# franioli/icepy4d

Measured on AMD Instinct MI355X. Metric: matched stereo image-pairs/sec (4096 kpts, 1080p), higher is better.
Workload: dtype f32

## Files before the change

icepy4d_amd/csrc/attention_bx.hip:

```cpp
#include "bf16x3.h"
#include "common.h"
#include "kernels.h"

namespace im {

static constexpr int BKT = 32;
static constexpr int BKS = 144;
static constexpr int BVS = 192;
static constexpr int BK_PLANE = BKT * BKS, BV_PLANE = BKT * BVS;
static constexpr int B_STAGE = 3 * BK_PLANE + 3 * BV_PLANE;
static constexpr int B_LDS = 2 * B_STAGE;
static constexpr int DPL = BKT * 128;
static constexpr int D_LDS = 3 * 3 * (DPL + DPL);

__device__ __forceinline__ f32x16 mfma_attn(u32x4 a, u32x4 b, f32x16 c) {
#ifdef BX_ABL_NO_MFMA
    c[0] += __uint_as_float(a.x ^ b.x);
    return c;
#else
    return mfma_bf(a, b, c);
#endif
}

typedef __attribute__((address_space(3))) bf16x4 lds_bf16x4;
// ... 449 lines not shown
        sc = sn;
        { const int rr = r0; r0 = r1; r1 = r2; r2 = RD == 3 ? rr : r0; }
        __syncthreads();
    }
    if (a.clock && nt > 8) {
        const unsigned long long ck1 = __builtin_amdgcn_s_memtime(), cr1 = __builtin_amdgcn_s_memrealtime();
        if (threadIdx.x == 0) {
            unsigned long long* cp = a.clock + 2 * (blockIdx.x % CLOCK_PROBE_SLOTS);
            cp[0] = ck1 - ck0; cp[1] = cr1 - cr0;
        }
    }
    {
        const int t = nt - 1;
        m_use = softmax_ref<true>(sc, t * BKT, nk, hh, m_run, l_run, o0, o1);
        softmax_exp(sc, m_use, l_run);
        pv_mul(r0, sc);
    }

    if (n_split > 1) {
        const long prow = (((long)z * a.heads + head) * a.n_max + min(qrow, a.n_max - 1)) * 66;
        const long pstride = (long)a.batch * a.heads * a.n_max * 66;
        float* pp = a.part + (long)split * pstride + prow;
        if (qrow < nq) {
#pragma unroll
            for (int g = 0; g < 4; ++g) {
                *reinterpret_cast<float2*>(pp + 8 * g + 4 * hh) = make_float2(o0[4 * g], o0[4 * g + 1]);
                *reinterpret_cast<float2*>(pp + 8 * g + 4 * hh + 2) = make_float2(o0[4 * g + 2], o0[4 * g + 3]);
                *reinterpret_cast<float2*>(pp + 32 + 8 * g + 4 * hh) = make_float2(o1[4 * g], o1[4 * g + 1]);
                *reinterpret_cast<float2*>(pp + 32 + 8 * g + 4 * hh + 2) = make_float2(o1[4 * g + 2], o1[4 * g + 3]);
            }
            if (hh == 0) { pp[64] = m_run; pp[65] = l_run; }
        }
        __threadfence();
        __syncthreads();
        int* flag = reinterpret_cast<int*>(bsm);
        if (tid == 0) {
            int* cnt = a.counters + ((long)z * a.heads + head) * nqb + qblk;
            const int old = atomicAdd(cnt, 1);
            *flag = (old == n_split - 1);
            if (old == n_split - 1) *cnt = 0;
        }
        __syncthreads();
        if (!*flag) return;
        __threadfence();
        float m = -INFINITY;
        for (int sidx = 0; sidx < n_split; ++sidx) m = fmaxf(m, a.part[(long)sidx * pstride + prow + 64]);
        l_run = 0.f;
#pragma unroll
        for (int r = 0; r < 16; ++r) { o0[r] = 0.f; o1[r] = 0.f; }
        for (int sidx = 0; sidx < n_split; ++sidx) {
            const float* ps = a.part + (long)sidx * pstride + prow;
            const float w = __builtin_amdgcn_exp2f(ps[64] - m);
            l_run += w * ps[65];
#pragma unroll
            for (int g = 0; g < 4; ++g)
#pragma unroll
                for (int q = 0; q < 4; ++q) {
                    o0[4 * g + q] += w * ps[8 * g + 4 * hh + q];
                    o1[4 * g + q] += w * ps[32 + 8 * g + 4 * hh + q];
                }
        }
    }

    if (qrow < nq) {
        const float inv = 1.f / l_run;
        float* op = a.out + (long)z * a.out_bstride + (long)qrow * a.ldo + head * 64;
#pragma unroll
        for (int g = 0; g < 4; ++g) {
            const float4 w0 = make_float4(o0[4 * g] * inv, o0[4 * g + 1] * inv, o0[4 * g + 2] * inv, o0[4 * g + 3] * inv);
            const float4 w1 = make_float4(o1[4 * g] * inv, o1[4 * g + 1] * inv, o1[4 * g + 2] * inv, o1[4 * g + 3] * inv);
            *reinterpret_cast<float4*>(op + 8 * g + 4 * hh) = w0;
            *reinterpret_cast<float4*>(op + 32 + 8 * g + 4 * hh) = w1;
        }
    }
}

hipError_t launch_attn_planes(const AttnArgs& a, hipStream_t s) {
    if (!a.planes || a.n_max <= 0 || attn_f32_form(a)) return hipSuccess;
    const long rows = (long)a.batch * a.heads * a.n_max;
    hipLaunchKernelGGL(kv_planes_kernel, dim3((unsigned)((rows + 31) / 32), 2), dim3(256), 0, s, a);
    return hipGetLastError();
}

hipError_t launch_flash_attn_bx(const AttnArgs& a, hipStream_t s) {
    const dim3 grid(((a.n_max + 127) / 128) * a.heads * a.batch * (a.part ? ATTN_MAX_SPLIT : 1)), block(256);
    static const bool reg_staging = env_int("IM_ATTN_REG_STAGING") != 0;
    if (a.planes && !reg_staging) return launch_dyn_lds<flash_attn_bx_kernel<true, true>>(grid, block, D_LDS, s, a);
    if (a.planes) return launch_dyn_lds<flash_attn_bx_kernel<true, false>>(grid, block, B_LDS, s, a);
    return launch_dyn_lds<flash_attn_bx_kernel<false, false>>(grid, block, B_LDS, s, a);
}

}
```

icepy4d_amd/csrc/block.h:

```cpp
#pragma once
#include "ctx.h"

namespace im {

struct BlockFfn {
    int act = 0;
    const float* w0 = nullptr; const float* w0p = nullptr;
    const float* b0 = nullptr;
    const float* ln_g = nullptr; const float* ln_b = nullptr;
    const float* w3 = nullptr; const float* w3p = nullptr;
    const float* b3 = nullptr;
    const char* name_fused = nullptr; const char* name_ffn0 = nullptr; const char* name_ffn3 = nullptr;
};

int launch_block_proj(im_ctx* ctx, hipStream_t s, const char* name, const GemmArgs& g, const float* wp_layers, int layer);

int launch_block_tail(im_ctx* ctx, hipStream_t s, const AttnArgs& at, const BlockFfn& f, const GemmArgs& base, float* x);

}
```

icepy4d_amd/csrc/block.hip:

```cpp
#include "block.h"

#include "lg_misc.h"
#include "workspace.h"

namespace im {

int launch_block_proj(im_ctx* ctx, hipStream_t s, const char* name, const GemmArgs& g, const float* wp_layers, int layer) {
    if (env_is_1("IM_PROJ_TILED")) {
        IM_LAUNCH(ctx, name, s, launch_gemm(g, s));
        return 0;
    }
    GemmArgs r = g;
    r.wp = reinterpret_cast<const unsigned char*>(wp_layers) + (size_t)layer * g.N * 256 * 6;
    IM_LAUNCH(ctx, name, s, launch_proj_rows(r, s));
    return 0;
}

int launch_block_tail(im_ctx* ctx, hipStream_t s, const AttnArgs& at, const BlockFfn& f, const GemmArgs& base, float* x) {
    Workspace* ws = ctx->ws;
    const long xb = (long)base.m_max * 256, hb = (long)base.m_max * 512;
    IM_LAUNCH(ctx, "attn_kv_planes", s, launch_attn_planes(at, s));
    IM_LAUNCH(ctx, at.cross ? "flash_attn_cross" : "flash_attn_self", s, launch_flash_attn(at, s));
    static const bool unfused = env_is_1("IM_FFN_UNFUSED");
    if (!unfused) {
        FfnArgs a;
        a.act = f.act; a.x = x; a.x_bstride = xb; a.att = at.out; a.att_bstride = xb;
        a.w0p = f.w0p; a.b0 = f.b0; a.ln_g = f.ln_g; a.ln_b = f.ln_b; a.w3p = f.w3p; a.b3 = f.b3;
        a.m_max = base.m_max; a.batch = base.batch; a.m_ptr = base.m_ptr; a.active = base.active; a.pstride = base.pstride;
        IM_LAUNCH(ctx, f.name_fused, s, launch_ffn_fused(a, s));
        return 0;
    }
    {
        GemmArgs g = base;
        g.A = x; g.a_bstride = xb; g.lda = 256; g.A1 = at.out; g.a1_bstride = xb; g.lda1 = 256; g.ksplit = 256;
        g.W = f.w0; g.ldw = 512; g.bias = f.b0; g.N = 512; g.K = 512;
        g.C = ws->h; g.c_bstride = hb; g.ldc = 512; g.epi = f.act == 1 ? EPI_BIAS_RELU : EPI_BIAS;
        IM_LAUNCH(ctx, f.name_ffn0, s, launch_gemm(g, s));
    }
    if (f.act == 0)
        IM_LAUNCH(ctx, "lg_layernorm_gelu", s, launch_layernorm_gelu(ws->h, hb, ws->st, base.batch, base.m_max, f.ln_g, f.ln_b, s));
    {
        GemmArgs g = base;
        g.A = ws->h; g.a_bstride = hb; g.lda = 512; g.W = f.w3; g.ldw = 512; g.bias = f.b3; g.N = 256; g.K = 512;
        g.C = x; g.c_bstride = xb; g.ldc = 256; g.R = x; g.r_bstride = xb; g.ldr = 256; g.epi = EPI_BIAS_RESID;
        IM_LAUNCH(ctx, f.name_ffn3, s, launch_gemm(g, s));
    }
    return 0;
}

}
```

icepy4d_amd/csrc/capi.hip:

```cpp
#include "ctx.h"
#include "lg_misc.h"
#include "sp_post.h"
#include "workspace.h"

#include <algorithm>
#include <cstdio>
#include <cstdlib>
#include <cstring>

using namespace im;

template <int N, typename F>
static hipError_t with_uploads(const float* const (&src)[N], const size_t (&sizes)[N], hipStream_t st, F&& launch) {
    float* d[N] = {};
    hipError_t e = hipSuccess;
    for (int i = 0; i < N && e == hipSuccess; ++i) {
        e = hipMalloc(&d[i], sizes[i] * sizeof(float));
        if (e == hipSuccess) e = hipMemcpy(d[i], src[i], sizes[i] * sizeof(float), hipMemcpyHostToDevice);
    }
    if (e == hipSuccess) e = launch(d);
    const hipError_t e2 = hipStreamSynchronize(st);
    for (int i = 0; i < N; ++i) hipFree(d[i]);
    return e != hipSuccess ? e : e2;
}
// ... 83 lines not shown
    ws->sim_ps = (((size_t)K * K + (size_t)K + 4) + 3) & ~(size_t)3;
    ws->vec_ps = ((size_t)K + 4 + 3) & ~(size_t)3;
    ws->part_ps = (size_t)((K + 15) / 16 + 1) * (K + 4);
    A(ws->sim, NP * ws->sim_ps + (size_t)K + 8);
    A(ws->sim2, (size_t)1);
    A(ws->rmax, NP * ws->vec_ps); A(ws->rlog, NP * ws->vec_ps); A(ws->cmax, NP * ws->vec_ps); A(ws->clog, NP * ws->vec_ps);
    A(ws->part, NP * ws->part_ps);
    A(ws->ridx, NP * ws->vec_ps); A(ws->rval, NP * ws->vec_ps); A(ws->cbest, NP * ws->vec_ps);
    A(ws->st, NP); A(ws->sel, NP + 3);
    A(ws->uv, (size_t)4 * (K + 8));
#undef A
    ws->n_pairs = (int)NP;
    if (!ok) {
        for (void* p : ws->allocs) ctx->gfree(p);
        delete ws;
        ctx->max_h = ctx->max_w = ctx->max_images = ctx->max_kpts = 0;
        return ctx->fail(-31, "im_ctx_reserve: out of device memory (%d x %d, %d images, %d keypoints)", max_h, max_w, max_images, max_kpts);
    }
    ctx->ws = ws;
    ctx->max_h = max_h; ctx->max_w = max_w; ctx->max_images = max_images; ctx->max_kpts = max_kpts;
    IM_HIP(ctx, hipMemset(ws->st, 0, sizeof(LGState) * NP));
    IM_HIP(ctx, hipMemset(ws->sel, 0, (NP + 3) * sizeof(int)));
    IM_HIP(ctx, hipMemset(ws->attn_cnt, 0, attn_counter_ints((int)K, (int)NI, 4) * sizeof(int)));
    IM_HIP(ctx, hipDeviceSynchronize());
    return 0;
}

int im_profile_begin(im_ctx* ctx) {
    IM_CHECK_CTX(ctx);
    IM_HIP(ctx, hipDeviceSynchronize());
    for (auto& e : ctx->prof) { ctx->prof_pool.push_back(e.e0); ctx->prof_pool.push_back(e.e1); }
    ctx->prof.clear();
    ctx->prof_on = true;
    return 0;
}

int im_profile_end(im_ctx* ctx, char* buf, size_t cap) {
    IM_CHECK_CTX(ctx);
    ctx->prof_on = false;
    constexpr int NCAL = 32;
    hipEvent_t cal[2 * NCAL];
    for (int i = 0; i < NCAL; ++i) {
        cal[2 * i] = ctx->prof_event(); cal[2 * i + 1] = ctx->prof_event();
        hipEventRecord(cal[2 * i], ctx->prof_stream);
        hipEventRecord(cal[2 * i + 1], ctx->prof_stream);
    }
    IM_HIP(ctx, hipDeviceSynchronize());
    std::map<std::string, std::pair<int, double>> agg;
    for (int i = 0; i < NCAL; ++i) {
        float ms = 0.f;
        if (hipEventElapsedTime(&ms, cal[2 * i], cal[2 * i + 1]) == hipSuccess) { agg["_empty_event_pair"].first += 1; agg["_empty_event_pair"].second += ms; }
        ctx->prof_pool.push_back(cal[2 * i]); ctx->prof_pool.push_back(cal[2 * i + 1]);
    }
    for (auto& e : ctx->prof) {
        float ms = 0.f;
        IM_HIP(ctx, hipEventElapsedTime(&ms, e.e0, e.e1));
        auto& a = agg[e.name];
        a.first += 1;
        a.second += ms;
    }
    std::string out = "{";
    bool first = true;
    for (auto& kv : agg) {
        char line[256];
        snprintf(line, sizeof(line), "%s\"%s\": {\"count\": %d, \"total_ms\": %.6f}", first ? "" : ", ", kv.first.c_str(),
                 kv.second.first, kv.second.second);
        out += line;
        first = false;
    }
    out += "}";
    if (!buf || out.size() + 1 > cap) return ctx->fail(-60, "im_profile_end: buffer too small (%zu needed)", out.size() + 1);
    memcpy(buf, out.c_str(), out.size() + 1);
    return 0;
}

int im_debug_read(im_ctx* ctx, const char* name, float* d_dst, size_t nfloats, void* stream) {
    IM_CHECK_CTX(ctx);
    Workspace* ws = ctx->ws;
    if (!ws || !name) return ctx->fail(-51, "im_debug_read: no workspace");
    const size_t K = (size_t)ctx->max_kpts;
    const std::string nm = name;
    const float* src = nullptr;
    size_t avail = 0;
    if (nm == "lg_x") { src = ws->x[ctx->dbg_cur]; avail = 2 * K * 256; }
    else if (nm == "lg_cos") { src = ws->cs[ctx->dbg_cur]; avail = 2 * K * 32; }
    else if (nm == "lg_sin") { src = ws->sn[ctx->dbg_cur]; avail = 2 * K * 32; }
    else if (nm == "sim") { src = ws->sim; avail = K * K; }
    else if (nm == "md") { src = ws->md; avail = 2 * K * 256; }
    else if (nm == "sp_smap") { src = ws->smap; avail = ws->smap_floats; }
    else if (nm == "sp_nms") { src = ws->nms; avail = ws->smap_floats; }
    else return ctx->fail(-61, "im_debug_read: unknown buffer '%s'", name);
    if (nfloats > avail) return ctx->fail(-62, "im_debug_read: %zu floats requested, %zu available", nfloats, avail);
    IM_HIP(ctx, hipMemcpyAsync(d_dst, src, nfloats * sizeof(float), hipMemcpyDeviceToDevice, (hipStream_t)stream));
    IM_HIP(ctx, hipStreamSynchronize((hipStream_t)stream));
    return 0;
}

int im_debug_clock_probe(im_ctx* ctx, int arm, double* h_out, void* stream) {
    IM_CHECK_CTX(ctx);
    hipStream_t s = (hipStream_t)stream;
    const size_t bytes = (size_t)CLOCK_PROBE_SLOTS * 2 * sizeof(unsigned long long);
    if (arm == 1) {
        IM_GROW(ctx, ctx->grow(ctx->scratch.clock[0], bytes, "clock_probe_attention"), -22, "im_debug_clock_probe: allocation failed");
        IM_GROW(ctx, ctx->grow(ctx->scratch.clock[1], bytes, "clock_probe_convolution"), -22, "im_debug_clock_probe: allocation failed");
        IM_HIP(ctx, hipMemsetAsync(ctx->scratch.clock[0].p, 0, bytes, s));
        IM_HIP(ctx, hipMemsetAsync(ctx->scratch.clock[1].p, 0, bytes, s));
        IM_HIP(ctx, hipStreamSynchronize(s));
        ctx->clock_armed = true;
        return 0;
    }
    if (!ctx->scratch.clock[0].p || !h_out) return ctx->fail(-51, "im_debug_clock_probe: not armed");
    std::vector<unsigned long long> h((size_t)CLOCK_PROBE_SLOTS * 2);
    const void* src[2] = {ctx->scratch.clock[0].p, ctx->scratch.clock[1].p};
    for (int c = 0; c < 2; ++c) {
        IM_HIP(ctx, hipMemcpyAsync(h.data(), src[c], bytes, hipMemcpyDeviceToHost, s));
        IM_HIP(ctx, hipStreamSynchronize(s));
        std::vector<double> mhz;
        for (int i = 0; i < CLOCK_PROBE_SLOTS; ++i)
            if (h[2 * i + 1] > 0) mhz.push_back(100.0 * (double)h[2 * i] / (double)h[2 * i + 1]);
        std::sort(mhz.begin(), mhz.end());
        h_out[2 * c] = mhz.empty() ? 0.0 : mhz[mhz.size() / 2];
        h_out[2 * c + 1] = (double)mhz.size();
    }
    if (arm == 0) ctx->clock_armed = false;
    return 0;
}

int im_gemm_nt(im_ctx* ctx, const float* d_a, const float* d_w, const float* d_bias, float* d_c, int m, int n, int k,
               float alpha, int big_tile, void* stream) {
    IM_CHECK_CTX(ctx);
    GemmArgs g;
    g.A = d_a; g.lda = k; g.W = d_w; g.ldw = k; g.bias = d_bias; g.N = n; g.K = k; g.m_max = m;
    g.C = d_c; g.ldc = n; g.alpha = alpha; g.epi = EPI_BIAS; g.big_tile = big_tile & 1; g.bx = (big_tile >> 1) & 1;
    IM_HIP(ctx, launch_gemm(g, (hipStream_t)stream));
    return 0;
}

int im_ffn_fused(im_ctx* ctx, int act, float* d_x, const float* d_att, const float* h_w0, const float* h_b0, const float* h_ln_g,
                   const float* h_ln_b, const float* h_w3, const float* h_b3, int n_images, int n_rows, const int32_t* d_n, void* stream) {
    IM_CHECK_CTX(ctx);
    if (n_images < 1 || n_rows < 1 || act < 0 || act > 1 || (act == 0 && (!h_ln_g || !h_ln_b))) return ctx->fail(-12, "im_ffn_fused: bad arguments");
    if (act == 1) h_ln_g = h_ln_b = h_b0;
    const std::vector<float> p0 = pack_frag_weights(h_w0, 512, 512), p3 = pack_frag_weights(h_w3, 256, 512);
    const size_t sizes[6] = {p0.size(), 512, 512, 512, p3.size(), 256};
    const float* src[6] = {p0.data(), h_b0, h_ln_g, h_ln_b, p3.data(), h_b3};
    hipStream_t st = (hipStream_t)stream;
    IM_HIP(ctx, with_uploads(src, sizes, st, [&](float* const* d) {
        FfnArgs f;
        f.act = act; f.x = d_x; f.x_bstride = (long)n_rows * 256; f.att = d_att; f.att_bstride = (long)n_rows * 256;
        f.w0p = d[0]; f.b0 = d[1]; f.ln_g = d[2]; f.ln_b = d[3]; f.w3p = d[4]; f.b3 = d[5];
        f.m_max = n_rows; f.batch = n_images; f.m_ptr = d_n; f.pstride = 2;
        return ctx->timed("ffn_fused", st, [&] { return launch_ffn_fused(f, st); });
    }));
    return 0;
}

static int conv3x3_entry(im_ctx* ctx, bool wino, const float* d_in, const float* h_weight, const float* h_bias, float* d_out,
                         int b, int h, int w, int cin, int cout, int relu, int pool, void* stream) {
    IM_CHECK_CTX(ctx);
    if (cin % 16 || cout % 64) return ctx->fail(-10, "im_conv3x3: cin %% 16 and cout %% 64 must be 0");
    std::vector<float> packed = wino ? pack_conv3x3_wino(h_weight, cout, cin) : pack_conv3x3(h_weight, cout, cin);
    std::vector<float> planes = wino ? pack_conv3x3_wino_bx(h_weight, cout, cin) : std::vector<float>(1);
    const size_t sizes[3] = {packed.size(), (size_t)cout, planes.size()};
    const float* src[3] = {packed.data(), h_bias, planes.data()};
    hipStream_t st = (hipStream_t)stream;
    IM_HIP(ctx, with_uploads(src, sizes, st, [&](float* const* d) {
        ConvArgs a;
        a.in = d_in; a.w = d[0]; a.bias = d[1]; a.out = d_out; a.B = b; a.H = h; a.W = w; a.Cin = cin; a.Cout = cout;
        a.relu = relu; a.pool = pool;
        if (wino) a.wx = d[2];
        return ctx->timed(wino ? "conv_wino" : "conv_direct", st, [&] { return wino ? launch_conv3x3_wino(a, st) : launch_conv3x3(a, st); });
    }));
    return 0;
// ... 88 lines not shown
```

icepy4d_amd/csrc/gemm.hip:

```cpp
#include "bf16x3.h"
#include "common.h"
#include "kernels.h"

namespace im {

template <int BM, int BN, int BK, int EPI, bool BX>
__global__ __launch_bounds__(256) void gemm_nt_kernel(GemmArgs a) {
    constexpr int LDS_LD = BK + 4;
    constexpr int WM = BM / 2, WN = BN / 2;
    constexpr int MB = WM / 32, NB = WN / 32;
    constexpr int F4 = BK / 4;
    constexpr int A_IT = BM * F4 / 256, B_IT = BN * F4 / 256;
    constexpr int XS = BK * 2 + 16, XPA = BM * XS, XPB = BN * XS;
    __shared__ __attribute__((aligned(16))) float smem[BX ? 3 * (XPA + XPB) / 4 : (BM + BN) * LDS_LD];
    float* sA = smem;
    float* sB = smem + BM * LDS_LD;
    unsigned char* const xA = reinterpret_cast<unsigned char*>(smem);
    unsigned char* const xB = xA + 3 * XPA;

    const int gm = (a.m_max + BM - 1) / BM;
    const int z = blockIdx.y;
    const int pair = a.pair_batched ? z : (z >> 1);
    if (a.active && a.active[pair * a.pstride] == 0) return;
    const int M = a.m_ptr ? a.m_ptr[a.pair_batched ? z * a.pstride : (z >> 1) * a.pstride + (z & 1)] : a.m_max;
// ... 133 lines not shown
        }
        __syncthreads();
    }
#undef IM_LOAD_SLAB
#undef IM_LD_A
#undef IM_LD_B
#undef IM_ST
#undef IM_ST_F32

    constexpr unsigned OOB = 0xFFFFF000u;
#pragma unroll
    for (int i = 0; i < MB; ++i)
#pragma unroll
        for (int j = 0; j < NB; ++j) {
            const int colbase = n0 + wn0 + j * 32;
            const int col = colbase + c;
            const bool col_ok = col < Nlive;
            const float bv = (bias && col_ok) ? bias[col] : 0.f;
            const unsigned rowl = m0 + wm0 + i * 32 + 4 * hh;
            if constexpr (EPI == EPI_BIAS || EPI == EPI_BIAS_RELU || EPI == EPI_BIAS_RESID) {
                const __amdgpu_buffer_rsrc_t rC = make_rsrc(a.C + (long)z * a.c_bstride, (unsigned)M * a.ldc * 4u);
                const unsigned vo = col_ok ? (rowl * a.ldc + col) * 4u : OOB;
                const unsigned rstep = (unsigned)a.ldc * 4u;
                float rv[16];
                if constexpr (EPI == EPI_BIAS_RESID) {
                    const __amdgpu_buffer_rsrc_t rR = make_rsrc(a.R + (long)z * a.r_bstride, (unsigned)M * a.ldr * 4u);
                    const unsigned vr = col_ok ? (rowl * a.ldr + col) * 4u : OOB;
#pragma unroll
                    for (int r = 0; r < 16; ++r)
                        rv[r] = __uint_as_float(__builtin_amdgcn_raw_buffer_load_b32(rR, vr, ((r & 3) + 8 * (r >> 2)) * (unsigned)a.ldr * 4u, 0));
                }
#pragma unroll
                for (int r = 0; r < 16; ++r) {
                    float val = acc[i][j][r] + bv;
                    if constexpr (EPI == EPI_BIAS) val = a.alpha * val;
                    else if constexpr (EPI == EPI_BIAS_RELU) val = fmaxf(val, 0.f);
                    else val = rv[r] + val;
                    __builtin_amdgcn_raw_buffer_store_b32(__float_as_uint(val), rC, vo, ((r & 3) + 8 * (r >> 2)) * rstep, 0);
                }
            } else {
                int which = 0, hd = colbase;
                if constexpr (EPI == EPI_QKV_ROPE || EPI == EPI_HEADS_QV) { which = colbase >> 8; hd = colbase & 255; }
                float* dst = a.q;
                if constexpr (EPI == EPI_QKV_ROPE) dst = which == 0 ? a.q : (which == 1 ? a.k : a.v);
                if constexpr (EPI == EPI_HEADS_QV) dst = which ? a.v : a.q;
                const __amdgpu_buffer_rsrc_t rD = make_rsrc(dst + (long)z * a.head_bstride + (long)(hd >> 6) * a.head_stride, (unsigned)M * 256u);
                const int d = (hd & 63) + c;
                const unsigned vo = col_ok ? (rowl * 64 + d) * 4u : OOB;
                float scale = a.alpha;
                if constexpr (EPI == EPI_QKV_ROPE) scale = 1.f;
                if constexpr (EPI == EPI_HEADS_QV) scale = which ? 1.f : a.alpha;
                const bool rope = EPI == EPI_QKV_ROPE && which < 2 && a.cs;
                if (rope) {
                    const __amdgpu_buffer_rsrc_t rCs = make_rsrc(a.cs + (long)z * a.enc_bstride, (unsigned)M * 128u);
                    const __amdgpu_buffer_rsrc_t rSn = make_rsrc(a.sn + (long)z * a.enc_bstride, (unsigned)M * 128u);
                    const unsigned ve = (rowl * 32 + (d >> 1)) * 4u;
#pragma unroll
                    for (int r = 0; r < 16; ++r) {
                        const unsigned so = ((r & 3) + 8 * (r >> 2)) * 128u;
                        const float cs = __uint_as_float(__builtin_amdgcn_raw_buffer_load_b32(rCs, ve, so, 0));
                        const float sn = __uint_as_float(__builtin_amdgcn_raw_buffer_load_b32(rSn, ve, so, 0));
                        const float val = acc[i][j][r] + bv;
                        const float partner = __shfl_xor(val, 1);
                        const float outv = (d & 1) ? (val * cs) + (partner * sn) : (val * cs) + ((-partner) * sn);
                        __builtin_amdgcn_raw_buffer_store_b32(__float_as_uint(outv), rD, vo, ((r & 3) + 8 * (r >> 2)) * 256u, 0);
                    }
                } else {
#pragma unroll
                    for (int r = 0; r < 16; ++r)
                        __builtin_amdgcn_raw_buffer_store_b32(__float_as_uint(scale * (acc[i][j][r] + bv)), rD, vo, ((r & 3) + 8 * (r >> 2)) * 256u, 0);
                }
            }
        }
}

namespace pr {
constexpr int BM = 32, NT = 512;
constexpr int PS = 528;
constexpr int PLANE = BM * PS;
constexpr int LDS_BYTES = 3 * PLANE;
constexpr unsigned TILE_BYTES = (256 / 16) * 3 * 1024;
}

#ifdef IM_PSTAMP
__device__ unsigned long long g_pstamp[4096 * 16];
#define P_STAMP(i) { if (wave == 0) { const unsigned long long ts_ = __builtin_amdgcn_s_memtime(); const int b_ = blockIdx.y * gridDim.x + blockIdx.x; if (lane == 0 && b_ < 4096) g_pstamp[b_ * 16 + (i)] = ts_; } }
extern "C" int im_debug_pstamps(unsigned long long* host, size_t n) {
    return (int)hipMemcpyFromSymbol(host, HIP_SYMBOL(g_pstamp), n * sizeof(unsigned long long));
}
#else
#define P_STAMP(i)
#endif

template <int EPI, int TILES>
__global__ __launch_bounds__(pr::NT, 4) void proj_rows_kernel(GemmArgs a) {
    using namespace pr;
    static_assert(EPI == EPI_QKV_ROPE || EPI == EPI_HEADS_QV, "the two projections of a LightGlue block");
    extern __shared__ __attribute__((aligned(16))) unsigned char psm[];
    const int z = blockIdx.y, pair = z >> 1;
    if (a.active && a.active[pair * a.pstride] == 0) return;
    const int M = a.m_ptr ? a.m_ptr[pair * a.pstride + (z & 1)] : a.m_max;
    const int m0 = blockIdx.x * BM;
    if (m0 >= M) return;
    const int tid = threadIdx.x, lane = tid & 63;
    const int wave = __builtin_amdgcn_readfirstlane(tid >> 6);
    const int c = lane & 31, hh = lane >> 5;
    const __amdgpu_buffer_rsrc_t rX = make_rsrc(a.A + (long)z * a.a_bstride, (unsigned)M * 1024u);
    const __amdgpu_buffer_rsrc_t rW = make_rsrc(a.wp, (unsigned)a.N * 256u * 6u);

    P_STAMP(0)
    u32x4 b0[3], b1[3], b2[3], b3[3];
#define PR_LOAD(b_, s_)                                                                                                          \
    {                                                                                                                            \
        const bool in_ = (s_) < TILES * 16;                                                                                      \
        const unsigned so_ = in_ ? (unsigned)((((s_) >> 4) * 8 + wave)) * TILE_BYTES + (unsigned)(((s_) & 15) * 3) * 1024u : 0u;   \
        const unsigned vo_ = in_ ? lane * 16u : 0x80000000u;     \
        _Pragma("unroll") for (int g = 0; g < 3; ++g) b_[g] = __builtin_amdgcn_raw_buffer_load_b128(rW, vo_, so_ + (unsigned)g * 1024u, 0); \
    }
    PR_LOAD(b0, 0)
    PR_LOAD(b1, 1)
    PR_LOAD(b2, 2)
    {
        float4 v[4];
#pragma unroll
        for (int i = 0; i < 4; ++i) {
            const int idx = tid + i * NT;
            v[i] = buf_load4(rX, (unsigned)((m0 + (idx >> 6)) * 256 + (idx & 63) * 4) * 4u, 0);
        }
#pragma unroll
        for (int i = 0; i < 4; ++i) {
            const int idx = tid + i * NT;
            unsigned h0, m0_, l0, h1, m1, l1;
            split2(v[i].x, v[i].y, h0, m0_, l0);
            split2(v[i].z, v[i].w, h1, m1, l1);
            unsigned char* d = psm + (idx >> 6) * PS + (idx & 63) * 8;
            *reinterpret_cast<u32x2*>(d) = u32x2{h0, h1};
            *reinterpret_cast<u32x2*>(d + PLANE) = u32x2{m0_, m1};
            *reinterpret_cast<u32x2*>(d + 2 * PLANE) = u32x2{l0, l1};
        }
    }
    __syncthreads();
    P_STAMP(1)

#define PR_SIX(b_, kc_)                                                                                              \
    {                                                                                                                \
        const unsigned char* ap = psm + c * PS + ((kc_) * 16 + hh * 8) * 2;                                          \
        const u32x4 ah = *reinterpret_cast<const u32x4*>(ap), am = *reinterpret_cast<const u32x4*>(ap + PLANE),   \
                     al = *reinterpret_cast<const u32x4*>(ap + 2 * PLANE);                                          \
        acc = mfma_bf(ah, b_[2], acc);                                                                              \
        acc = mfma_bf(al, b_[0], acc);                                                                              \
        acc = mfma_bf(am, b_[1], acc);                                                                              \
        acc = mfma_bf(ah, b_[1], acc);                                                                              \
        acc = mfma_bf(am, b_[0], acc);                                                                              \
        acc = mfma_bf(ah, b_[0], acc);                                                                              \
    }
#pragma unroll 1
    for (int j = 0; j < TILES; ++j) {
        const int tile = j * 8 + wave;
        f32x16 acc;
#pragma unroll
        for (int r = 0; r < 16; ++r) acc[r] = 0.f;
#pragma unroll 1
        for (int kc = 0; kc < 16; kc += 4) {
            const int s_ = j * 16 + kc;
            PR_LOAD(b3, s_ + 3)
            __builtin_amdgcn_sched_barrier(0);
            PR_SIX(b0, kc)
            __builtin_amdgcn_sched_barrier(0);
            PR_LOAD(b0, s_ + 4)
            __builtin_amdgcn_sched_barrier(0);
            PR_SIX(b1, kc + 1)
            __builtin_amdgcn_sched_barrier(0);
            PR_LOAD(b1, s_ + 5)
            __builtin_amdgcn_sched_barrier(0);
            PR_SIX(b2, kc + 2)
            __builtin_amdgcn_sched_barrier(0);
            PR_LOAD(b2, s_ + 6)
            __builtin_amdgcn_sched_barrier(0);
            PR_SIX(b3, kc + 3)
            __builtin_amdgcn_sched_barrier(0);
        }
        P_STAMP(2 + 2 * j)
        const int colbase = tile * 32;
        const int col = colbase + c;
        const float bv = a.bias ? a.bias[col] : 0.f;
        const unsigned rowl = m0 + 4 * hh;
        const int which = colbase >> 8, hd = colbase & 255;
        float* dst = a.q;
        if constexpr (EPI == EPI_QKV_ROPE) dst = which == 0 ? a.q : (which == 1 ? a.k : a.v);
        if constexpr (EPI == EPI_HEADS_QV) dst = which ? a.v : a.q;
        const __amdgpu_buffer_rsrc_t rD = make_rsrc(dst + (long)z * a.head_bstride + (long)(hd >> 6) * a.head_stride, (unsigned)M * 256u);
        const int d = (hd & 63) + c;
        const unsigned vo = (rowl * 64 + d) * 4u;
        float scale = a.alpha;
        if constexpr (EPI == EPI_QKV_ROPE) scale = 1.f;
        if constexpr (EPI == EPI_HEADS_QV) scale = which ? 1.f : a.alpha;
        const bool rope = EPI == EPI_QKV_ROPE && which < 2 && a.cs;
        if (rope) {
            const __amdgpu_buffer_rsrc_t rCs = make_rsrc(a.cs + (long)z * a.enc_bstride, (unsigned)M * 128u);
            const __amdgpu_buffer_rsrc_t rSn = make_rsrc(a.sn + (long)z * a.enc_bstride, (unsigned)M * 128u);
            const unsigned ve = (rowl * 32 + (d >> 1)) * 4u;
#pragma unroll
            for (int r = 0; r < 16; ++r) {
                const unsigned so = ((r & 3) + 8 * (r >> 2)) * 128u;
                const float cs = __uint_as_float(__builtin_amdgcn_raw_buffer_load_b32(rCs, ve, so, 0));
                const float sn = __uint_as_float(__builtin_amdgcn_raw_buffer_load_b32(rSn, ve, so, 0));
                const float val = acc[r] + bv;
                const float partner = __shfl_xor(val, 1);
                const float outv = (d & 1) ? (val * cs) + (partner * sn) : (val * cs) + ((-partner) * sn);
                __builtin_amdgcn_raw_buffer_store_b32(__float_as_uint(outv), rD, vo, ((r & 3) + 8 * (r >> 2)) * 256u, 0);
            }
        } else {
#pragma unroll
            for (int r = 0; r < 16; ++r)
                __builtin_amdgcn_raw_buffer_store_b32(__float_as_uint(scale * (acc[r] + bv)), rD, vo, ((r & 3) + 8 * (r >> 2)) * 256u, 0);
        }
        P_STAMP(3 + 2 * j)
    }
#undef PR_LOAD
#undef PR_SIX
}

template <int EPI, int TILES>
static hipError_t launch_proj_rows_t(const GemmArgs& a, hipStream_t s) {
    const dim3 grid((a.m_max + pr::BM - 1) / pr::BM, a.batch), block(pr::NT);
    return launch_dyn_lds<proj_rows_kernel<EPI, TILES>>(grid, block, pr::LDS_BYTES, s, a);
}

hipError_t launch_proj_rows(const GemmArgs& a, hipStream_t s) {
    if (!a.wp || a.K != 256 || a.lda != 256 || a.A1 || a.sel || a.w_bstride || a.n_ptr || a.pair_batched) return hipErrorInvalidValue;
    if (a.m_max <= 0 || a.batch <= 0) return hipSuccess;
    if (a.epi == EPI_QKV_ROPE && a.N == 768) return launch_proj_rows_t<EPI_QKV_ROPE, 3>(a, s);
    if (a.epi == EPI_HEADS_QV && a.N == 512) return launch_proj_rows_t<EPI_HEADS_QV, 2>(a, s);
    return hipErrorInvalidValue;
}

hipError_t launch_gemm(const GemmArgs& a, hipStream_t s) {
    if (a.K % 32 != 0 || (a.A1 && a.ksplit % 64 != 0)) return hipErrorInvalidValue;
    const int bm = a.big_tile ? 128 : 64, bn = bm;
    dim3 grid(((a.N + bn - 1) / bn) * ((a.m_max + bm - 1) / bm), a.batch), block(256);
    if (grid.x == 0) return hipSuccess;
#define IM_GEMM_CASE(E)                                                                  \
    case E:                                                                              \
        if (a.bx) {                                                                      \
            if (a.big_tile) hipLaunchKernelGGL((gemm_nt_kernel<128, 128, 32, E, true>), grid, block, 0, s, a);   \
            else hipLaunchKernelGGL((gemm_nt_kernel<64, 64, 32, E, true>), grid, block, 0, s, a);               \
        } else {                                                                         \
            if (a.big_tile) hipLaunchKernelGGL((gemm_nt_kernel<128, 128, 32, E, false>), grid, block, 0, s, a);  \
            else hipLaunchKernelGGL((gemm_nt_kernel<64, 64, 32, E, false>), grid, block, 0, s, a);              \
        }                                                                                \
        break;
    switch (a.epi) {
        IM_GEMM_CASE(EPI_BIAS)
        IM_GEMM_CASE(EPI_BIAS_RESID)
        IM_GEMM_CASE(EPI_HEADS)
        IM_GEMM_CASE(EPI_QKV_ROPE)
        IM_GEMM_CASE(EPI_BIAS_RELU)
        IM_GEMM_CASE(EPI_HEADS_QV)
        default: return hipErrorInvalidValue;
    }
#undef IM_GEMM_CASE
    return hipGetLastError();
}

}
```

icepy4d_amd/csrc/kernels.h:

```cpp
#pragma once
#include <hip/hip_runtime.h>
#include <stdint.h>
#include <cstdlib>
#include <vector>

#include "common.h"

namespace im {

inline bool env_is_1(const char* name) {
    const char* e = getenv(name);
    return e && e[0] == '1';
}
inline int env_int(const char* name) {
    const char* e = getenv(name);
    return e ? atoi(e) : 0;
}

inline hipError_t current_device(int* dev) {
    if (hipError_t e = hipGetDevice(dev); e != hipSuccess) return e;
    return (*dev < 0 || *dev >= IM_MAX_DEVICES) ? hipErrorInvalidDevice : hipSuccess;
}
inline hipError_t device_cu_count(int* n) {
    static int n_cu[IM_MAX_DEVICES] = {0};
    int dev = 0;
    if (hipError_t e = current_device(&dev); e != hipSuccess) return e;
    if (!n_cu[dev]) {
        if (hipError_t e = hipDeviceGetAttribute(&n_cu[dev], hipDeviceAttributeMultiprocessorCount, dev); e != hipSuccess) return e;
    }
    *n = n_cu[dev];
    return hipSuccess;
}
template <auto Kernel>
hipError_t optin_dyn_lds(size_t bytes) {
    static size_t have[IM_MAX_DEVICES] = {0};
    int dev = 0;
    if (hipError_t e = current_device(&dev); e != hipSuccess) return e;
    if (bytes > have[dev]) {
        if (hipError_t e = hipFuncSetAttribute(reinterpret_cast<const void*>(Kernel), hipFuncAttributeMaxDynamicSharedMemorySize, (int)bytes); e != hipSuccess) return e;
        have[dev] = bytes;
    }
    return hipSuccess;
}
template <auto Kernel, typename... Args>
hipError_t launch_dyn_lds(dim3 grid, dim3 block, size_t lds_bytes, hipStream_t s, const Args&... args) {
    if (hipError_t e = optin_dyn_lds<Kernel>(lds_bytes); e != hipSuccess) return e;
    hipLaunchKernelGGL(Kernel, grid, block, lds_bytes, s, args...);
    return hipGetLastError();
}

enum GemmEpi {
    EPI_BIAS = 0,
    EPI_BIAS_RESID = 1,
    EPI_HEADS = 2,
    EPI_QKV_ROPE = 3,
    EPI_BIAS_RELU = 4,
    EPI_HEADS_QV = 5,
};

struct GemmArgs {
    const float* A = nullptr;  long a_bstride = 0;  int lda = 0;
    const float* A1 = nullptr; long a1_bstride = 0; int lda1 = 0; int ksplit = 0;
    const float* W = nullptr;  int ldw = 0; long w_bstride = 0;
    const float* bias = nullptr;
    const int* sel = nullptr; long w_sel_stride = 0; long bias_sel_stride = 0;
    int N = 0, K = 0;
    int m_max = 0;
    const int* m_ptr = nullptr;
    const int* n_ptr = nullptr;
    const int* active = nullptr;
    int pstride = 2;
    int pair_batched = 0;
    int batch = 1;
    float alpha = 1.f;
    float* C = nullptr; long c_bstride = 0; int ldc = 0;
    const float* R = nullptr; long r_bstride = 0; int ldr = 0;
    float* q = nullptr; float* k = nullptr; float* v = nullptr; long head_bstride = 0; long head_stride = 0;
    const float* cs = nullptr; const float* sn = nullptr; long enc_bstride = 0;
    int epi = EPI_BIAS;
    int big_tile = 0;
    int bx = 0;
    const void* wp = nullptr;
};
hipError_t launch_gemm(const GemmArgs& a, hipStream_t s);
hipError_t launch_proj_rows(const GemmArgs& a, hipStream_t s);

struct FfnArgs {
    int act = 0;
    float* x = nullptr; long x_bstride = 0;
    const float* att = nullptr; long att_bstride = 0;
    const float* w0p = nullptr; const float* b0 = nullptr;
    const float* ln_g = nullptr; const float* ln_b = nullptr;
    const float* w3p = nullptr; const float* b3 = nullptr;
    int m_max = 0; int batch = 1;
    const int* m_ptr = nullptr;
    const int* active = nullptr;
    int pstride = 2;
};
hipError_t launch_ffn_fused(const FfnArgs& a, hipStream_t s);
std::vector<float> pack_frag_weights(const float* w, int n, int k);

struct AttnArgs {
    const float* q = nullptr; const float* k = nullptr; const float* v = nullptr;
    long bstride = 0; long hstride = 0;
    float* out = nullptr; long out_bstride = 0; int ldo = 256;
    const int* n_ptr = nullptr;
    int pstride = 2;
    int n_max = 0; int batch = 2; int heads = 4; int cross = 0;
    float scale = 1.f;
    const int* active = nullptr;
    float* part = nullptr;
    int* counters = nullptr;
    void* planes = nullptr;
    int f32_form = 0;
    unsigned long long* clock = nullptr;
};
static constexpr int CLOCK_PROBE_SLOTS = 4096;
static constexpr int ATTN_MAX_SPLIT = 4;
inline size_t attn_part_floats(int n_max, int batch, int heads) { return (size_t)ATTN_MAX_SPLIT * batch * heads * n_max * 66; }
inline size_t attn_planes_bytes(int n_max, int batch, int heads) { return (size_t)2 * batch * heads * n_max * 384; }
inline size_t attn_counter_ints(int n_max, int batch, int heads) { return (size_t)batch * heads * ((n_max + 127) / 128); }
bool attn_f32_form(const AttnArgs& a);
hipError_t launch_flash_attn(const AttnArgs& a, hipStream_t s);
hipError_t launch_attn_planes(const AttnArgs& a, hipStream_t s);
hipError_t launch_flash_attn_bx(const AttnArgs& a, hipStream_t s);

struct ConvArgs {
    const float* in = nullptr;
    const float* w = nullptr;
    const float* bias = nullptr;
    float* out = nullptr;
    int B = 1, H = 0, W = 0, Cin = 0, Cout = 0;
    int pool = 0;
    int relu = 1;
    const uint8_t* img = nullptr;
    int img_channels = 1;
    int gray_mode = 0;
    const float* w1 = nullptr;
    const float* b1 = nullptr;
    const float* w1q = nullptr;
    const void* wx = nullptr;
    int f32_form = 0;
    unsigned long long* clock = nullptr;
};
hipError_t launch_conv3x3(const ConvArgs& a, hipStream_t s);
hipError_t launch_conv3x3_wino(const ConvArgs& a, hipStream_t s);
hipError_t launch_conv3x3_wino_bx2(const ConvArgs& a, hipStream_t s);
hipError_t launch_conv1a(const uint8_t* img, int channels, int gray_mode, const float* w, const float* bias, float* out, int B, int H,
                         int W, hipStream_t s);

}
```

icepy4d_amd/csrc/lightglue.hip:

```cpp
#include "block.h"
#include "lg_misc.h"
#include "workspace.h"

using namespace im;

static constexpr int ST_INTS = (int)(sizeof(LGState) / sizeof(int));

static int lg_block(im_ctx* ctx, hipStream_t s, int NI, int layer, bool cross, float* x, const float* cs, const float* sn) {
    Workspace* ws = ctx->ws;
    const LightGlueW& W = ctx->lg;
    const int K = ctx->max_kpts;
    const long xb = (long)K * 256;
    const int* n_ptr = ws->st->n;
    const int* active = &ws->st->active;
    GemmArgs base;
    base.m_max = K; base.m_ptr = n_ptr; base.active = active; base.pstride = ST_INTS; base.batch = NI; base.bx = 1;
    AttnArgs at;
    at.q = ws->q; at.k = cross ? ws->q : ws->k; at.v = ws->v; at.hstride = (long)K * 64; at.bstride = (long)K * 256;
    at.out = ws->att; at.out_bstride = xb; at.ldo = 256; at.n_ptr = n_ptr; at.pstride = ST_INTS; at.n_max = K; at.batch = NI; at.heads = 4;
    at.cross = cross ? 1 : 0; at.active = active; at.part = ws->attn_part; at.counters = ws->attn_cnt; at.planes = ws->attn_planes; at.clock = ctx->clock_of(0);
    GemmArgs g = base;
    g.A = x; g.a_bstride = xb; g.lda = 256; g.ldw = 256; g.K = 256;
    g.q = ws->q; g.v = ws->v; g.head_bstride = (long)K * 256; g.head_stride = (long)K * 64; g.big_tile = NI >= 4;
    if (!cross) {
        g.W = W.qkv_w + (long)layer * 768 * 256; g.bias = W.qkv_b + (long)layer * 768; g.N = 768; g.epi = EPI_QKV_ROPE;
        g.k = ws->k; g.cs = cs; g.sn = sn; g.enc_bstride = (long)K * 32;
        if (int rc = launch_block_proj(ctx, s, "lg_qkv_rope_gemm", g, W.qkv_wp, layer)) return rc;
        at.scale = 0.125f;
    } else {
        g.W = W.cqv_w + (long)layer * 512 * 256; g.bias = W.cqv_b + (long)layer * 512; g.N = 512; g.epi = EPI_HEADS_QV;
        g.alpha = (float)0.35355339059327373;
        if (int rc = launch_block_proj(ctx, s, "lg_proj_gemm", g, W.cqv_wp, layer)) return rc;
        at.scale = 1.f;
    }
    const LightGlueW::Ffn& F = cross ? W.cross_ffn : W.self_ffn;
    BlockFfn f;
    f.w0 = F.w0 + (long)layer * 512 * 512; f.w0p = F.w0p + (long)layer * 512 * 512 * 3 / 2; f.b0 = F.b0 + (long)layer * 512;
    f.ln_g = F.ln_g + (long)layer * 512; f.ln_b = F.ln_b + (long)layer * 512;
    f.w3 = F.w3 + (long)layer * 256 * 512; f.w3p = F.w3p + (long)layer * 256 * 512 * 3 / 2; f.b3 = F.b3 + (long)layer * 256;
    f.name_fused = "lg_ffn_fused"; f.name_ffn0 = "lg_ffn0_gemm"; f.name_ffn3 = "lg_ffn3_gemm";
    return launch_block_tail(ctx, s, at, f, base, x);
}

static int lightglue_forward(im_ctx* ctx, int n_pairs, const float* d_kpts, const float* d_desc, const int32_t* d_n, const float* h_size,
                             const im_lightglue_conf* conf, int32_t* d_matches, float* d_mscores, int32_t* d_prune, int32_t* d_info,
                             void* stream) {
    IM_CHECK_CTX(ctx);
    if (!ctx->lg.ready) return ctx->fail(-50, "im_lightglue_forward: weights not finalized");
    Workspace* ws = ctx->ws;
    if (!ws) return ctx->fail(-51, "im_lightglue_forward: call im_ctx_reserve first");
    if (n_pairs < 1 || n_pairs > ws->n_pairs || n_pairs > 64)
        return ctx->fail(-53, "im_lightglue_forward: %d pairs, the workspace was reserved for %d (max_images / 2)", n_pairs, ws->n_pairs);
    hipStream_t s = (hipStream_t)stream;
    const LightGlueW& W = ctx->lg;
    const int K = ctx->max_kpts;
    const int L = conf->n_layers;
    const int NP = n_pairs, NI = 2 * n_pairs;
    if (L < 1 || L > 9) return ctx->fail(-52, "im_lightglue_forward: n_layers must be 1..9");
    const bool do_stop = conf->depth_confidence > 0, do_prune = conf->width_confidence > 0;
    const long xb = (long)K * 256, eb = (long)K * 32;
    LGState* st = ws->st;

    IM_HIP(ctx, launch_lg_init(st, NI, d_n, ws->ind[0], ws->prune, K, K, d_matches, d_mscores, K, s));
    IM_HIP(ctx, hipMemcpyAsync(ws->x[0], d_desc, sizeof(float) * NI * xb, hipMemcpyDeviceToDevice, s));
    IM_HIP(ctx, launch_posenc(d_kpts, (long)K * 2, st, NI, K, W.wr, h_size, ws->cs[0], ws->sn[0], eb, s));
    int cur = 0;
    for (int i = 0; i < L; ++i) {
        int rc = lg_block(ctx, s, NI, i, false, ws->x[cur], ws->cs[cur], ws->sn[cur]);
        if (rc) return rc;
        rc = lg_block(ctx, s, NI, i, true, ws->x[cur], ws->cs[cur], ws->sn[cur]);
        if (rc) return rc;
        if (i == L - 1) break;
        if (!do_stop && !do_prune) continue;
        IM_LAUNCH(ctx, "lg_adapt", s, launch_rowdot(ws->x[cur], xb, st, NI, K, do_stop ? W.tc_w + (long)i * 256 : nullptr, W.tc_b + i, 1,
                                  do_prune ? W.ma_w + (long)i * 256 : nullptr, W.ma_b + i, nullptr, ws->conf, ws->msc, K,
                                  W.thr[i], do_stop ? i : -1, 1, s));
        const float keep_thr = (float)(1.0 - (double)conf->width_confidence);
        IM_LAUNCH(ctx, "lg_adapt", s, launch_stop_prune(st, NP, i, do_stop, do_prune, (float)conf->depth_confidence, keep_thr, W.thr[i], ws->conf,
                                                      ws->msc, K, ws->ind[cur], ws->ind[1 - cur], ws->keep_idx, ws->prune, K,
                                                      conf->pruning_min_kpts, s));
        if (do_prune) {
            IM_LAUNCH(ctx, "lg_adapt", s, launch_gather_rows(st, NI, K, ws->keep_idx, K, ws->x[cur], ws->x[1 - cur], xb, ws->cs[cur], ws->cs[1 - cur],
                                                           ws->sn[cur], ws->sn[1 - cur], eb, do_stop ? i : -1, (float)conf->depth_confidence, s));
            cur = 1 - cur;
        }
    }
    ctx->dbg_cur = cur;
    IM_HIP(ctx, launch_lg_select_layer(st, NP, L, ws->sel, d_info, s));
    {
        GemmArgs g;
        g.m_max = K; g.m_ptr = st->n; g.pstride = ST_INTS; g.batch = NI; g.bx = 1;
        g.A = ws->x[cur]; g.a_bstride = xb; g.lda = 256; g.W = W.fp_w; g.ldw = 256; g.bias = W.fp_b;
        g.sel = ws->sel; g.w_sel_stride = 65536; g.bias_sel_stride = 256; g.N = 256; g.K = 256;
        g.C = ws->md; g.c_bstride = xb; g.ldc = 256; g.alpha = 0.25f;
        g.epi = EPI_BIAS;
        IM_LAUNCH(ctx, "lg_proj_gemm", s, launch_gemm(g, s));
    }
    IM_HIP(ctx, launch_rowdot(ws->x[cur], xb, st, NI, K, W.ma_w, W.ma_b, 0, nullptr, nullptr, ws->sel, ws->z, nullptr, K, 0.f, -1, 0, s));
    IM_HIP(ctx, launch_logsig(ws->z, K, st, NI, K, ws->lz, s));
    {
        GemmArgs g;
        g.m_max = K; g.m_ptr = &st->n[0]; g.n_ptr = &st->n[1]; g.pstride = ST_INTS; g.pair_batched = 1; g.batch = NP; g.bx = 1;
        g.A = ws->md; g.a_bstride = 2 * xb; g.lda = 256; g.W = ws->md + xb; g.w_bstride = 2 * xb; g.ldw = 256; g.N = K; g.K = 256;
        g.C = ws->sim; g.c_bstride = (long)ws->sim_ps; g.ldc = K; g.epi = EPI_BIAS; g.big_tile = 1;
        IM_LAUNCH(ctx, "score_gemm", s, launch_gemm(g, s));
    }
    AssignArgs a;
    a.sim = ws->sim; a.ld = K; a.m_ptr = &st->n[0]; a.n_ptr = &st->n[1]; a.m_max = K; a.n_max = K;
    a.lz0 = ws->lz; a.lz1 = ws->lz + K;
    a.rmax = ws->rmax; a.rlog = ws->rlog; a.cmax = ws->cmax; a.clog = ws->clog; a.part = ws->part;
    a.ridx = ws->ridx; a.rval = ws->rval; a.cbest = ws->cbest; a.threshold = (float)conf->filter_threshold;
    a.ind0 = ws->ind[cur]; a.ind1 = ws->ind[cur] + K;
    a.out_m0 = d_matches; a.out_m1 = d_matches + K; a.out_s0 = d_mscores; a.out_s1 = d_mscores + K;
    a.n_pairs = NP; a.sim_ps = (long)ws->sim_ps; a.vec_ps = (long)ws->vec_ps; a.part_ps = (long)ws->part_ps; a.lz_ps = 2L * K;
    a.out_ps = 2L * K; a.state_ps = ST_INTS;
// ... 38 lines not shown
```

Baseline: 170.5.

## Fuse K/V bf16x3 plane packing into projection GEMM epilogue

The projection GEMM epilogue now splits K and V outputs into bf16x3 planes directly, using a DPP lane swap to pair adjacent columns. The separate attn_kv_planes kernel is skipped when the planes were already filled. K/V f32 outputs are no longer stored when planes are written. This removes one kernel launch and a full re-read of K/V per layer, in exchange for extra epilogue stores and a heavier epilogue inside the GEMM. The debug-read buffers were also extended.

```diff
diff --git a/icepy4d_amd/csrc/attention_bx.hip b/icepy4d_amd/csrc/attention_bx.hip
--- a/icepy4d_amd/csrc/attention_bx.hip
+++ b/icepy4d_amd/csrc/attention_bx.hip
@@ -555,9 +555,16 @@
     return hipGetLastError();
 }
 
+static bool attn_reg_staging() {
+    static const bool env = env_int("IM_ATTN_REG_STAGING") != 0;
+    return env;
+}
+
+bool attn_product_form(const AttnArgs& a) { return a.planes && !attn_f32_form(a) && !attn_reg_staging(); }
+
 hipError_t launch_flash_attn_bx(const AttnArgs& a, hipStream_t s) {
     const dim3 grid(((a.n_max + 127) / 128) * a.heads * a.batch * (a.part ? ATTN_MAX_SPLIT : 1)), block(256);
-    static const bool reg_staging = env_int("IM_ATTN_REG_STAGING") != 0;
+    const bool reg_staging = attn_reg_staging();
     if (a.planes && !reg_staging) return launch_dyn_lds<flash_attn_bx_kernel<true, true>>(grid, block, D_LDS, s, a);
     if (a.planes) return launch_dyn_lds<flash_attn_bx_kernel<true, false>>(grid, block, B_LDS, s, a);
     return launch_dyn_lds<flash_attn_bx_kernel<false, false>>(grid, block, B_LDS, s, a);
diff --git a/icepy4d_amd/csrc/block.h b/icepy4d_amd/csrc/block.h
--- a/icepy4d_amd/csrc/block.h
+++ b/icepy4d_amd/csrc/block.h
@@ -13,7 +13,7 @@
     const char* name_fused = nullptr; const char* name_ffn0 = nullptr; const char* name_ffn3 = nullptr;
 };
 
-int launch_block_proj(im_ctx* ctx, hipStream_t s, const char* name, const GemmArgs& g, const float* wp_layers, int layer);
+int launch_block_proj(im_ctx* ctx, hipStream_t s, const char* name, const GemmArgs& g, const float* wp_layers, int layer, AttnArgs* at = nullptr);
 
 int launch_block_tail(im_ctx* ctx, hipStream_t s, const AttnArgs& at, const BlockFfn& f, const GemmArgs& base, float* x);
 
diff --git a/icepy4d_amd/csrc/block.hip b/icepy4d_amd/csrc/block.hip
--- a/icepy4d_amd/csrc/block.hip
+++ b/icepy4d_amd/csrc/block.hip
@@ -5,13 +5,19 @@
 
 namespace im {
 
-int launch_block_proj(im_ctx* ctx, hipStream_t s, const char* name, const GemmArgs& g, const float* wp_layers, int layer) {
+int launch_block_proj(im_ctx* ctx, hipStream_t s, const char* name, const GemmArgs& g, const float* wp_layers, int layer, AttnArgs* at) {
+    if (at) at->planes_filled = 0;
     if (env_is_1("IM_PROJ_TILED")) {
         IM_LAUNCH(ctx, name, s, launch_gemm(g, s));
         return 0;
     }
     GemmArgs r = g;
     r.wp = reinterpret_cast<const unsigned char*>(wp_layers) + (size_t)layer * g.N * 256 * 6;
+    if (at && attn_product_form(*at) && !env_is_1("IM_KV_PLANES_PASS")) {
+        r.planes = static_cast<unsigned char*>(at->planes);
+        r.planes_v_ofs = (long)at->batch * at->heads * at->n_max * 384;
+        at->planes_filled = 1;
+    }
     IM_LAUNCH(ctx, name, s, launch_proj_rows(r, s));
     return 0;
 }
@@ -19,7 +25,7 @@
 int launch_block_tail(im_ctx* ctx, hipStream_t s, const AttnArgs& at, const BlockFfn& f, const GemmArgs& base, float* x) {
     Workspace* ws = ctx->ws;
     const long xb = (long)base.m_max * 256, hb = (long)base.m_max * 512;
-    IM_LAUNCH(ctx, "attn_kv_planes", s, launch_attn_planes(at, s));
+    if (!at.planes_filled) IM_LAUNCH(ctx, "attn_kv_planes", s, launch_attn_planes(at, s));
     IM_LAUNCH(ctx, at.cross ? "flash_attn_cross" : "flash_attn_self", s, launch_flash_attn(at, s));
     static const bool unfused = env_is_1("IM_FFN_UNFUSED");
     if (!unfused) {
diff --git a/icepy4d_amd/csrc/capi.hip b/icepy4d_amd/csrc/capi.hip
--- a/icepy4d_amd/csrc/capi.hip
+++ b/icepy4d_amd/csrc/capi.hip
@@ -189,13 +189,15 @@
     const std::string nm = name;
     const float* src = nullptr;
     size_t avail = 0;
-    if (nm == "lg_x") { src = ws->x[ctx->dbg_cur]; avail = 2 * K * 256; }
+    if (nm == "lg_x") { src = ws->x[ctx->dbg_cur]; avail = (size_t)2 * ws->n_pairs * K * 256; }
     else if (nm == "lg_cos") { src = ws->cs[ctx->dbg_cur]; avail = 2 * K * 32; }
     else if (nm == "lg_sin") { src = ws->sn[ctx->dbg_cur]; avail = 2 * K * 32; }
     else if (nm == "sim") { src = ws->sim; avail = K * K; }
     else if (nm == "md") { src = ws->md; avail = 2 * K * 256; }
     else if (nm == "sp_smap") { src = ws->smap; avail = ws->smap_floats; }
     else if (nm == "sp_nms") { src = ws->nms; avail = ws->smap_floats; }
+    else if (nm == "lg_q") { src = ws->q; avail = (size_t)2 * ws->n_pairs * K * 256; }
+    else if (nm == "attn_planes") { src = reinterpret_cast<const float*>(ws->attn_planes); avail = attn_planes_bytes((int)K, 2 * ws->n_pairs, 4) / 4; }
     else return ctx->fail(-61, "im_debug_read: unknown buffer '%s'", name);
     if (nfloats > avail) return ctx->fail(-62, "im_debug_read: %zu floats requested, %zu available", nfloats, avail);
     IM_HIP(ctx, hipMemcpyAsync(d_dst, src, nfloats * sizeof(float), hipMemcpyDeviceToDevice, (hipStream_t)stream));
diff --git a/icepy4d_amd/csrc/gemm.hip b/icepy4d_amd/csrc/gemm.hip
--- a/icepy4d_amd/csrc/gemm.hip
+++ b/icepy4d_amd/csrc/gemm.hip
@@ -239,6 +239,10 @@
 constexpr unsigned TILE_BYTES = (256 / 16) * 3 * 1024;
 }
 
+__device__ __forceinline__ float lane_xor1(float x) {
+    return __int_as_float(__builtin_amdgcn_update_dpp(0, __float_as_int(x), 0xB1, 0xF, 0xF, true));
+}
+
 #ifdef IM_PSTAMP
 __device__ unsigned long long g_pstamp[4096 * 16];
 #define P_STAMP(i) { if (wave == 0) { const unsigned long long ts_ = __builtin_amdgcn_s_memtime(); const int b_ = blockIdx.y * gridDim.x + blockIdx.x; if (lane == 0 && b_ < 4096) g_pstamp[b_ * 16 + (i)] = ts_; } }
@@ -346,31 +350,56 @@
         float* dst = a.q;
         if constexpr (EPI == EPI_QKV_ROPE) dst = which == 0 ? a.q : (which == 1 ? a.k : a.v);
         if constexpr (EPI == EPI_HEADS_QV) dst = which ? a.v : a.q;
-        const __amdgpu_buffer_rsrc_t rD = make_rsrc(dst + (long)z * a.head_bstride + (long)(hd >> 6) * a.head_stride, (unsigned)M * 256u);
+        const long hofs = (long)z * a.head_bstride + (long)(hd >> 6) * a.head_stride;
+        const __amdgpu_buffer_rsrc_t rD = make_rsrc(dst + hofs, (unsigned)M * 256u);
         const int d = (hd & 63) + c;
         const unsigned vo = (rowl * 64 + d) * 4u;
         float scale = a.alpha;
         if constexpr (EPI == EPI_QKV_ROPE) scale = 1.f;
         if constexpr (EPI == EPI_HEADS_QV) scale = which ? 1.f : a.alpha;
+        const bool kv_planes = a.planes && (EPI == EPI_HEADS_QV || which > 0);
+        const bool f32_out = !a.planes || which == 0;
         const bool rope = EPI == EPI_QKV_ROPE && which < 2 && a.cs;
+        const int kv = EPI == EPI_QKV_ROPE ? max(which - 1, 0) : which;
+        const __amdgpu_buffer_rsrc_t rP = make_rsrc(a.planes + (long)kv * a.planes_v_ofs + hofs * 6, kv_planes ? (unsigned)M * 384u : 0u);
+        const bool odd = d & 1;
+        const unsigned vp = (rowl + (odd ? 1u : 0u)) * 384u + (unsigned)(d & ~1) * 2u;
+        auto put2 = [&](int r, float o0, float o1) {
+            if (f32_out) {
+                __builtin_amdgcn_raw_buffer_store_b32(__float_as_uint(o0), rD, vo, ((r & 3) + 8 * (r >> 2)) * 256u, 0);
+                __builtin_amdgcn_raw_buffer_store_b32(__float_as_uint(o1), rD, vo, ((r & 3) + 8 * (r >> 2) + 1) * 256u, 0);
+            }
+            if (kv_planes) {
+                const float other = lane_xor1(odd ? o0 : o1);
+                unsigned h, m, l;
+                split2(odd ? other : o0, odd ? o1 : other, h, m, l);
+                const unsigned so = ((r & 3) + 8 * (r >> 2)) * 384u;
+                __builtin_amdgcn_raw_buffer_store_b32(h, rP, vp, so, 0);
+                __builtin_amdgcn_raw_buffer_store_b32(m, rP, vp, so + 128u, 0);
+                __builtin_amdgcn_raw_buffer_store_b32(l, rP, vp, so + 256u, 0);
+            }
+        };
         if (rope) {
             const __amdgpu_buffer_rsrc_t rCs = make_rsrc(a.cs + (long)z * a.enc_bstride, (unsigned)M * 128u);
             const __amdgpu_buffer_rsrc_t rSn = make_rsrc(a.sn + (long)z * a.enc_bstride, (unsigned)M * 128u);
             const unsigned ve = (rowl * 32 + (d >> 1)) * 4u;
-#pragma unroll
-            for (int r = 0; r < 16; ++r) {
+            auto rot = [&](int r) {
                 const unsigned so = ((r & 3) + 8 * (r >> 2)) * 128u;
                 const float cs = __uint_as_float(__builtin_amdgcn_raw_buffer_load_b32(rCs, ve, so, 0));
                 const float sn = __uint_as_float(__builtin_amdgcn_raw_buffer_load_b32(rSn, ve, so, 0));
                 const float val = acc[r] + bv;
                 const float partner = __shfl_xor(val, 1);
-                const float outv = (d & 1) ? (val * cs) + (partner * sn) : (val * cs) + ((-partner) * sn);
-                __builtin_amdgcn_raw_buffer_store_b32(__float_as_uint(outv), rD, vo, ((r & 3) + 8 * (r >> 2)) * 256u, 0);
+                return (d & 1) ? (val * cs) + (partner * sn) : (val * cs) + ((-partner) * sn);
+            };
+#pragma unroll
+            for (int r = 0; r < 16; r += 4) {
+                const float o0 = rot(r), o1 = rot(r + 1), o2 = rot(r + 2), o3 = rot(r + 3);
+                put2(r, o0, o1);
+                put2(r + 2, o2, o3);
             }
         } else {
 #pragma unroll
-            for (int r = 0; r < 16; ++r)
-                __builtin_amdgcn_raw_buffer_store_b32(__float_as_uint(scale * (acc[r] + bv)), rD, vo, ((r & 3) + 8 * (r >> 2)) * 256u, 0);
+            for (int r = 0; r < 16; r += 2) put2(r, scale * (acc[r] + bv), scale * (acc[r + 1] + bv));
         }
         P_STAMP(3 + 2 * j)
     }
@@ -387,6 +416,8 @@
 hipError_t launch_proj_rows(const GemmArgs& a, hipStream_t s) {
     if (!a.wp || a.K != 256 || a.lda != 256 || a.A1 || a.sel || a.w_bstride || a.n_ptr || a.pair_batched) return hipErrorInvalidValue;
     if (a.m_max <= 0 || a.batch <= 0) return hipSuccess;
+    if (a.planes && (a.head_stride != (long)a.m_max * 64 || a.head_bstride != 4 * a.head_stride || a.planes_v_ofs != (long)a.batch * a.head_bstride * 6))
+        return hipErrorInvalidValue;
     if (a.epi == EPI_QKV_ROPE && a.N == 768) return launch_proj_rows_t<EPI_QKV_ROPE, 3>(a, s);
     if (a.epi == EPI_HEADS_QV && a.N == 512) return launch_proj_rows_t<EPI_HEADS_QV, 2>(a, s);
     return hipErrorInvalidValue;
diff --git a/icepy4d_amd/csrc/kernels.h b/icepy4d_amd/csrc/kernels.h
--- a/icepy4d_amd/csrc/kernels.h
+++ b/icepy4d_amd/csrc/kernels.h
@@ -81,6 +81,8 @@
     int big_tile = 0;
     int bx = 0;
     const void* wp = nullptr;
+    unsigned char* planes = nullptr;
+    long planes_v_ofs = 0;
 };
 hipError_t launch_gemm(const GemmArgs& a, hipStream_t s);
 hipError_t launch_proj_rows(const GemmArgs& a, hipStream_t s);
@@ -112,6 +114,7 @@
     float* part = nullptr;
     int* counters = nullptr;
     void* planes = nullptr;
+    int planes_filled = 0;
     int f32_form = 0;
     unsigned long long* clock = nullptr;
 };
@@ -123,6 +126,7 @@
 bool attn_f32_form(const AttnArgs& a);
 hipError_t launch_flash_attn(const AttnArgs& a, hipStream_t s);
 hipError_t launch_attn_planes(const AttnArgs& a, hipStream_t s);
+bool attn_product_form(const AttnArgs& a);
 hipError_t launch_flash_attn_bx(const AttnArgs& a, hipStream_t s);
 
 struct ConvArgs {
diff --git a/icepy4d_amd/csrc/lightglue.hip b/icepy4d_amd/csrc/lightglue.hip
--- a/icepy4d_amd/csrc/lightglue.hip
+++ b/icepy4d_amd/csrc/lightglue.hip
@@ -25,12 +25,12 @@
     if (!cross) {
         g.W = W.qkv_w + (long)layer * 768 * 256; g.bias = W.qkv_b + (long)layer * 768; g.N = 768; g.epi = EPI_QKV_ROPE;
         g.k = ws->k; g.cs = cs; g.sn = sn; g.enc_bstride = (long)K * 32;
-        if (int rc = launch_block_proj(ctx, s, "lg_qkv_rope_gemm", g, W.qkv_wp, layer)) return rc;
+        if (int rc = launch_block_proj(ctx, s, "lg_qkv_rope_gemm", g, W.qkv_wp, layer, &at)) return rc;
         at.scale = 0.125f;
     } else {
         g.W = W.cqv_w + (long)layer * 512 * 256; g.bias = W.cqv_b + (long)layer * 512; g.N = 512; g.epi = EPI_HEADS_QV;
         g.alpha = (float)0.35355339059327373;
-        if (int rc = launch_block_proj(ctx, s, "lg_proj_gemm", g, W.cqv_wp, layer)) return rc;
+        if (int rc = launch_block_proj(ctx, s, "lg_proj_gemm", g, W.cqv_wp, layer, &at)) return rc;
         at.scale = 1.f;
     }
     const LightGlueW::Ffn& F = cross ? W.cross_ffn : W.self_ffn;
```

Measured after the change: 171.2, median of 5. About the same (+0.4%).
